# Komputerowe-Projektowanie-Lekow/pmarlo

Measured on AMD Instinct MI355X. Metric: frames/sec featurize->TICA->k-means->T-matrix, 1Mx64 synth; ITS rel-err, higher is better.
Workload: dtype f64; 1 GPU; synthetic 1000000 frames x 64 f32 features per GPU (AR(1) latents), TICA->10, k=500 (10 Lloyd iterations), lag=10, row-normalised T; frames_per_gpu=1000000, features=64, tica_dim=10, k=500, lag=10, kmeans_iters=10, parallelism=shards1

## Files before the change

### pmarlo_amd/csrc/kmeans.hip

```cpp
#include "common.h"
#include "wave.h"

#include <algorithm>
#include <cstdlib>

namespace {

constexpr int kThreads = 256;

template <typename T>
__device__ __forceinline__ double load_as_f64(const T* p) { return (double)(*p); }

struct FitState {
    double scale;
    double inv_scale;
    double absmax;
    double shift2;
    double tol2;
    double done;
    double n_iter;
    double inertia;
};

__device__ __forceinline__ long long to_fixed(double v, double scale) { return __double2ll_rn(v * scale); }
// ... 748 lines not shown
}

__global__ void mfma_f16_probe_kernel(const uint16_t* __restrict__ A, const uint16_t* __restrict__ B,
                                      const float* __restrict__ C, float* __restrict__ D) {
    const int l = threadIdx.x, i = l & 15, q = l >> 4;
    A += (size_t)blockIdx.x * 512;
    B += (size_t)blockIdx.x * 512;
    C += (size_t)blockIdx.x * 256;
    D += (size_t)blockIdx.x * 256;
    v8h a, b;
    for (int j = 0; j < 8; ++j) {
        a[j] = __builtin_bit_cast(_Float16, A[i * 32 + 8 * q + j]);
        b[j] = __builtin_bit_cast(_Float16, B[(8 * q + j) * 16 + i]);
    }
    v4f32 c;
    for (int r = 0; r < 4; ++r) c[r] = C[(4 * q + r) * 16 + i];
    c = __builtin_amdgcn_mfma_f32_16x16x32_f16(a, b, c, 0, 0, 0);
    for (int r = 0; r < 4; ++r) D[(4 * q + r) * 16 + i] = c[r];
}

bool filter_enabled() {
    static const bool on = [] {
        const char* e = getenv("MSM_KMEANS_FILTER");
        return !(e && e[0] == '0');
    }();
    return on;
}

size_t filter_image_bytes(int64_t n, int) { return (size_t)((n + 63) & ~(int64_t)63) * 16 * kFilterRowQ + 16; }

template <typename T>
msm_status launch_pack(msm_ctx* ctx, const T* x, int64_t n, int d, int64_t ld, const double* mean, const double* stdv,
                       const double* absmax, uint4* image) {
    const unsigned grid = (unsigned)((n + 255) / 256);
    if (!absmax) {
        uint4* tail = image + (size_t)((n + 63) & ~(int64_t)63) * kFilterRowQ;
        MSM_HIP(ctx, hipMemsetAsync(tail, 0, 8, ctx->stream));
        const int g = (int)std::min<int64_t>((n * d + 256 * 8 - 1) / (256 * 8), (int64_t)ctx->n_cu * 8);
        hipLaunchKernelGGL(filter_absmax_kernel<T>, dim3(g), dim3(256), 0, ctx->stream, x, n, d, ld, mean, stdv,
                           (unsigned long long*)tail);
        MSM_CHECK_LAUNCH(ctx);
        absmax = (const double*)tail;
    }
    const int dense = ld == d && ((uintptr_t)x & 15) == 0;
#define MSM_PACK_CASE(D)                                                                                              \
    case D:                                                                                                           \
        hipLaunchKernelGGL((kmeans_pack_kernel<T, D>), dim3(grid), dim3(256), 0, ctx->stream, x, n, ld, mean, stdv, absmax, \
                           image, dense);                                                                             \
        break
    switch (d) {
        MSM_PACK_CASE(1); MSM_PACK_CASE(2); MSM_PACK_CASE(3); MSM_PACK_CASE(4); MSM_PACK_CASE(5);
        MSM_PACK_CASE(6); MSM_PACK_CASE(7); MSM_PACK_CASE(8); MSM_PACK_CASE(9); MSM_PACK_CASE(10);
        default: return msm_fail(ctx, MSM_ERR_UNSUPPORTED, "k-means frame images need d <= %d (got %d)", kFilterMaxD, d);
    }
#undef MSM_PACK_CASE
    MSM_CHECK_LAUNCH(ctx);
    return MSM_OK;
}

msm_status filter_stats_buffer(msm_ctx* ctx, unsigned long long** out) {
    static_assert(sizeof(unsigned long long) == 8, "");
    if (!ctx->km_stats) {
        if (ctx->capturing) { *out = nullptr; return MSM_OK; }
        MSM_HIP(ctx, hipMalloc(&ctx->km_stats, 16));
        MSM_HIP(ctx, hipMemsetAsync(ctx->km_stats, 0, 16, ctx->stream));
    }
    *out = (unsigned long long*)ctx->km_stats;
    return MSM_OK;
}

template <typename T, int DP, bool ACCUM>
msm_status launch_filter_dp(msm_ctx* ctx, const T* x, int64_t n, int d, int64_t ld, const double* centers, int k,
                            const double* mean, const double* stdv, const uint4* image, int32_t* labels, double* mindist,
                            const FitState* st, unsigned long long* sums, unsigned long long* counts, double* upd_centers) {
    constexpr int NF = 4;
    const size_t lds = filter_lds_bytes(k, d, ACCUM);
    msm_status rs;
    const int64_t n_units = (n + 16 * NF - 1) / (16 * NF);
    const int kWaves = filter_waves(DP, ACCUM, sizeof(T) == 8 && !mean);
    const int grid = (int)std::min<int64_t>((n_units + kWaves - 1) / kWaves, (int64_t)ctx->n_cu);
    unsigned long long* stats = nullptr;
    rs = filter_stats_buffer(ctx, &stats);
    if (rs != MSM_OK) return rs;
    auto kern = mean ? kmeans_filter_kernel<T, DP, NF, ACCUM, true> : kmeans_filter_kernel<T, DP, NF, ACCUM, false>;
    if (lds > 48 * 1024)
        MSM_HIP(ctx, hipFuncSetAttribute((const void*)kern, hipFuncAttributeMaxDynamicSharedMemorySize, (int)lds));
    hipLaunchKernelGGL(kern, dim3(grid), dim3(64 * kWaves), lds, ctx->stream, x, n, d, ld, k, mean, stdv, image, centers,
                       labels, mindist, st, sums, counts, stats, stats ? upd_centers : nullptr,
                       stats ? (unsigned int*)(stats + 1) : nullptr);
    MSM_CHECK_LAUNCH(ctx);
    return MSM_OK;
}

template <typename T, bool ACCUM>
msm_status launch_filter(msm_ctx* ctx, const T* x, int64_t n, int d, int64_t ld, const double* centers, int k,
                         const double* mean, const double* stdv, const uint4* image, int32_t* labels, double* mindist,
                         const FitState* st, unsigned long long* sums, unsigned long long* counts, double* upd_centers) {
    if (filter_dp(d) == 4)
        return launch_filter_dp<T, 4, ACCUM>(ctx, x, n, d, ld, centers, k, mean, stdv, image, labels, mindist, st, sums,
                                             counts, upd_centers);
    return launch_filter_dp<T, 10, ACCUM>(ctx, x, n, d, ld, centers, k, mean, stdv, image, labels, mindist, st, sums, counts,
                                          upd_centers);
}

bool filter_fits(int k, int d, bool accum) { return filter_enabled() && d <= kFilterMaxD && filter_lds_bytes(k, d, accum) != 0; }

template <typename T, bool ACCUM>
msm_status dispatch_mfma(msm_ctx* ctx, const T* x, int64_t n, int d, int64_t ld, const double* centers, int k,
                         const double* mean, const double* stdv, int32_t* labels, double* mindist, const FitState* st,
                         unsigned long long* sums, unsigned long long* counts, const void* image = nullptr,
                         double* upd_centers = nullptr, bool* folded = nullptr) {
    if (folded) *folded = false;
    if (filter_fits(k, d, ACCUM)) {
        if (getenv("MSM_KMEANS_DEBUG"))
            fprintf(stderr, "msm_kmeans: filter T=%s n=%lld d=%d k=%d ACCUM=%d\n", sizeof(T) == 4 ? "f32" : "f64", (long long)n,
                    d, k, (int)ACCUM);
        if (!image) {
            msm_status rs = msm_reserve_km_image(ctx, filter_image_bytes(n, d));
            if (rs != MSM_OK) return rs;
            rs = launch_pack<T>(ctx, x, n, d, ld, mean, stdv, nullptr, (uint4*)ctx->km_image);
            if (rs != MSM_OK) return rs;
            image = ctx->km_image;
        }
        if (upd_centers && !(ACCUM && (int64_t)k * d <= kUpdateWide && (ctx->km_stats || !ctx->capturing))) upd_centers = nullptr;
        if (folded) *folded = upd_centers != nullptr;
        return launch_filter<T, ACCUM>(ctx, x, n, d, ld, centers, k, mean, stdv, (const uint4*)image, labels, mindist, st,
                                       sums, counts, upd_centers);
    }
#define MSM_MFMA_CASE(KSV) \
    if (d <= 4 * KSV)      \
        return launch_mfma<T, KSV, ACCUM>(ctx, x, n, d, ld, centers, k, mean, stdv, labels, mindist, st, sums, counts)
    MSM_MFMA_CASE(1);
    MSM_MFMA_CASE(2);
    MSM_MFMA_CASE(3);
    MSM_MFMA_CASE(4);
    MSM_MFMA_CASE(6);
    MSM_MFMA_CASE(8);
    MSM_MFMA_CASE(12);
    MSM_MFMA_CASE(16);
    MSM_MFMA_CASE(24);
    MSM_MFMA_CASE(32);
    MSM_MFMA_CASE(48);
    MSM_MFMA_CASE(64);
#undef MSM_MFMA_CASE
    return msm_fail(ctx, MSM_ERR_UNSUPPORTED, "k-means: d=%d > 256 not supported", d);
}

msm_status mfma_probe(msm_ctx* ctx, bool f16, const uint16_t* h_a, const uint16_t* h_b, const float* h_c, float* h_d,
                      int n_tiles) {
    if (!ctx) return MSM_ERR_INVALID;
    MSM_REQUIRE(ctx, n_tiles >= 1 && h_a && h_b && h_c && h_d, "msm_mfma_probe: bad arguments");
    const size_t na = (size_t)n_tiles * 512 * sizeof(uint16_t), nc = (size_t)n_tiles * 256 * sizeof(float);
    msm_status rs = msm_reserve_scratch(ctx, 2 * na + 2 * nc);
    if (rs != MSM_OK) return rs;
    unsigned char* base = (unsigned char*)ctx->scratch;
    uint16_t* d_a = (uint16_t*)base;
    uint16_t* d_b = (uint16_t*)(base + na);
    float* d_c = (float*)(base + 2 * na);
    float* d_d = (float*)(base + 2 * na + nc);
    MSM_HIP(ctx, hipMemcpyAsync(d_a, h_a, na, hipMemcpyHostToDevice, ctx->stream));
    MSM_HIP(ctx, hipMemcpyAsync(d_b, h_b, na, hipMemcpyHostToDevice, ctx->stream));
    MSM_HIP(ctx, hipMemcpyAsync(d_c, h_c, nc, hipMemcpyHostToDevice, ctx->stream));
    if (f16)
        hipLaunchKernelGGL(mfma_f16_probe_kernel, dim3((unsigned)n_tiles), dim3(64), 0, ctx->stream, d_a, d_b, d_c, d_d);
    else
        hipLaunchKernelGGL(mfma_bf16_probe_kernel, dim3((unsigned)n_tiles), dim3(64), 0, ctx->stream, d_a, d_b, d_c, d_d);
    MSM_CHECK_LAUNCH(ctx);
    MSM_HIP(ctx, hipMemcpyAsync(h_d, d_d, nc, hipMemcpyDeviceToHost, ctx->stream));
    MSM_HIP(ctx, hipStreamSynchronize(ctx->stream));
    return MSM_OK;
}

// ... 251 lines not shown
```

### pmarlo_amd/csrc/kmeans_filter.h

```cpp
#pragma once

typedef __bf16 v8bf __attribute__((ext_vector_type(8)));
typedef _Float16 v8h __attribute__((ext_vector_type(8)));
typedef float v4f32 __attribute__((ext_vector_type(4)));

#ifdef MSM_KMF_WAVES
__host__ __device__ constexpr int filter_waves(int, bool, bool) { return MSM_KMF_WAVES; }
#else
__host__ __device__ constexpr int filter_waves(int dp, bool heavy, bool plain) { return dp == 10 && heavy && !plain ? 12 : 16; }
#endif
constexpr int kFilterMaxD = 10;
constexpr int kFilterRowQ = 3;
constexpr double kFilterHi = 1e18;
constexpr double kFilterScaledHi = 16384.0;
constexpr double kF16MinNormal = 6.103515625e-05;
constexpr int kFilterScaleTop = 13;
constexpr double kFilterKappa = 52.0 * 5.9604644775390625e-08;
constexpr float kPickEps = 20.0f * 5.9604644775390625e-08f;
constexpr float kPickFloor = 1e-30f;
constexpr float kUp20 = 1.0f + 9.5367431640625e-07f;
constexpr double kUp20d = 1.0 + 9.5367431640625e-07;

__host__ __device__ inline int filter_scale_exp(double amax) {
    if (!(amax > 0.0) || !(amax <= 1.7976931348623157e308)) return 0;
// ... 157 lines not shown
    auto slot_addr = [&](int i, int sl) { return ((sl >> 3) * 16 + i) * 8 + (sl & 7); };
#pragma unroll
    for (int u = 0; u < kStageRegs; ++u) {
        const int i = lane + 64 * u;
        const int r = stage_row(i, d), f = i - r * d, j = tile * 16 + r;
        if (i < 16 * d && j < k) {
            tab[(size_t)j * S::RF + f] = (float)c[u];
            const double w = ldexp(c[u], ec);
            if (fabs(w) <= kFilterScaledHi) {
                unsigned short ch, cl;
                double tiny = 0.0;
                f16_split2(w, ch, cl, tiny);
                simg[slot_addr(r, filter_slot(0, f))] = ch;
                simg[slot_addr(r, filter_slot(1, f))] = ch;
                simg[slot_addr(r, filter_slot(2, f))] = cl;
            }
        }
    }
    __builtin_amdgcn_fence(__ATOMIC_ACQ_REL, "wavefront");
    int bad_row = 0;
    if (lane < 16) {
        const int j = tile * 16 + lane;
        float* row = tab + (size_t)j * S::RF;
        double h = __builtin_inf();
        if (j < k) {
            double a = 0.0, aw = 0.0, tiny = 0.0;
            bool ok = true;
#pragma unroll
            for (int f = 0; f < DP; ++f) {
                const double cf = rc[f];
                a = fma(cf, cf, a);
                const double w = ldexp(cf, ec);
                ok = ok && fabs(cf) <= kFilterHi && fabs(w) <= kFilterScaledHi;
                if (ok) {
                    aw = fma(w, w, aw);
                    const double r = fabs(w) >= kF16MinNormal ? fabs(w - f16_round(w)) : fabs(w);
                    if (!(r >= kF16MinNormal) || !(fabs(w) >= kF16MinNormal)) tiny += r;
                }
            }
            h = 0.5 * a;
            const double cval = ldexp(-(h - kFilterKappa * h), exc);
            ok = ok && fabs(cval) <= 0x1p100;
            if (!ok) bad_row = 1;
            cz[j] = ok ? f32_up(cval) : 0.0f;
            if (ok)
                simg[slot_addr(lane, kFilterSlotNorm)] =
                    f16_bits(f16_ceil(fmax((kFilterKappa * sqrt(aw) + 2.0 * tiny) * kUp20d, kF16MinNormal)));
            row[DP] = (float)h;
            row[DP + 1] = (float)(sqrt(a) * kUp20d);
        } else {
            cz[j] = -3.0e38f;
            row[DP] = 3.0e38f;
            row[DP + 1] = -3.0e38f;
        }
        hs[j] = h;
    }
    const bool bad = __any(bad_row != 0);
    if (bad && lane == 0) atomicOr(any_bad, 1);
}


template <typename T>
__global__ __launch_bounds__(256) void filter_absmax_kernel(const T* __restrict__ x, int64_t n, int d, int64_t ld,
                                                           const double* __restrict__ mean, const double* __restrict__ stdv,
                                                           unsigned long long* __restrict__ out_bits) {
    double m = 0.0;
    for (int64_t i = (int64_t)blockIdx.x * 256 + threadIdx.x; i < n * d; i += (int64_t)gridDim.x * 256) {
        const int64_t r = i / d;
        const int f = (int)(i - r * d);
        double v = load_as_f64(x + r * ld + f);
        if (mean) v = (v - mean[f]) / stdv[f];
        if (fabs(v) <= kFilterHi) m = fmax(m, fabs(v));
    }
    m = wave_max_f64(m);
    __shared__ double wm[4];
    if ((threadIdx.x & 63) == 0) wm[threadIdx.x >> 6] = m;
    __syncthreads();
    if (threadIdx.x == 0) {
        m = fmax(fmax(wm[0], wm[1]), fmax(wm[2], wm[3]));
        if (m > 0.0) atomicMax(out_bits, (unsigned long long)__double_as_longlong(m));
    }
}

template <typename T, int DP, bool WHITEN>
__device__ __forceinline__ void filter_load_frame(const T* __restrict__ x, int64_t ld, int d, bool vec_rows,
                                                  const double* __restrict__ mean, const double* __restrict__ stdv,
                                                  int64_t t, double (&z)[DP]) {
    const T* row = x + t * ld;
    if (vec_rows) {
        const double2* r2 = reinterpret_cast<const double2*>(row);
#pragma unroll
        for (int f2 = 0; f2 < DP / 2; ++f2) {
            const double2 v = r2[f2];
            z[2 * f2] = v.x;
            z[2 * f2 + 1] = v.y;
        }
    } else {
#pragma unroll
        for (int f = 0; f < DP; ++f) {
            const double v = load_as_f64(row + (f < d ? f : d - 1));
            z[f] = f < d ? v : 0.0;
        }
    }
    if constexpr (WHITEN) {
#pragma unroll
        for (int f = 0; f < DP; ++f) {
            const int fc = f < d ? f : d - 1;
            const double w = (z[f] - mean[fc]) / stdv[fc];
            z[f] = f < d ? w : 0.0;
        }
    }
}

template <int MT>
__device__ __forceinline__ void filter_close_iteration(const unsigned long long* sums, const unsigned long long* counts, int k,
                                                       int d, double* centers, FitState* st) {
    __shared__ double red[16];
    const int tid = threadIdx.x;
    const double inv_scale = st->inv_scale;
    for (int v0 = 0; v0 < 1024; v0 += MT) {
        const int v = v0 + tid;
        if (v < 1024) {
            double acc = 0.0;
            constexpr int CH = 4;
            for (int i0 = v; i0 < k * d; i0 += 1024 * CH) {
                long long cnt[CH], sm[CH];
                double old[CH];
#pragma unroll
                for (int c = 0; c < CH; ++c) {
                    const int i = i0 + c * 1024;
                    cnt[c] = 0;
                    if (i < k * d) {
                        cnt[c] = (long long)__hip_atomic_load(&counts[i / d], __ATOMIC_RELAXED, __HIP_MEMORY_SCOPE_AGENT);
                        sm[c] = (long long)__hip_atomic_load(&sums[i], __ATOMIC_RELAXED, __HIP_MEMORY_SCOPE_AGENT);
                        old[c] = centers[i];
                    }
                }
#pragma unroll
                for (int c = 0; c < CH; ++c)
                    if (cnt[c] > 0) {
                        const double c_new = (double)sm[c] * inv_scale / (double)cnt[c];
                        const double dlt = c_new - old[c];
                        acc = fma(dlt, dlt, acc);
                        centers[i0 + c * 1024] = c_new;
                    }
            }
            for (int off = 32; off > 0; off >>= 1) acc += __shfl_down(acc, off, 64);
            if ((v & 63) == 0) red[v >> 6] = acc;
        }
    }
    __syncthreads();
    if (tid == 0) {
        double t = 0.0;
        for (int i = 0; i < 16; ++i) t += red[i];
        st->shift2 = t;
        st->n_iter += 1.0;
        if (t <= st->tol2) st->done = 1.0;
    }
}

template <typename T, int DP, int NF, bool ACCUM, bool WHITEN>
__global__ __launch_bounds__(64 * filter_waves(DP, ACCUM, sizeof(T) == 8 && !WHITEN)) void kmeans_filter_kernel(
    const T* __restrict__ x, int64_t n, int d, int64_t ld, int k, const double* __restrict__ mean,
    const double* __restrict__ stdv, const uint4* __restrict__ image, const double* __restrict__ centers,
    int32_t* __restrict__ labels,
    double* __restrict__ mindist, const FitState* __restrict__ st, unsigned long long* __restrict__ sums,
    unsigned long long* __restrict__ counts, unsigned long long* __restrict__ n_scanned, double* upd_centers,
    unsigned int* __restrict__ ticket) {
    using S = FilterShape<DP>;
    constexpr int kFilterWaves = filter_waves(DP, ACCUM, sizeof(T) == 8 && !WHITEN);
    constexpr int kMT = 64 * kFilterWaves, RF = S::RF, RQ = kFilterRowQ;
    constexpr bool kReloadZ = ACCUM && DP == 10;
    static_assert(NF == 4, "one frame group per lane quarter: a unit is 64 frames, one per lane in the candidate pick");
    extern __shared__ __attribute__((aligned(16))) unsigned char smem_raw[];
    if constexpr (ACCUM) {
        if (st->done != 0.0) return;
    }
    const int k16 = (k + 15) & ~15;
    const int n_tiles = ((k16 / 16) + 1) & ~1;
    uint4* img = reinterpret_cast<uint4*>(smem_raw);
    float* tab = reinterpret_cast<float*>(img + (size_t)n_tiles * 64);
    float* cz = tab + (size_t)n_tiles * 16 * RF;
    double* hs = reinterpret_cast<double*>(cz + (size_t)n_tiles * 16);
    unsigned long long* lsum = reinterpret_cast<unsigned long long*>(hs + (size_t)n_tiles * 16);
    unsigned long long* lcnt = lsum + (ACCUM ? (size_t)k * d : 0);
    __shared__ int unit_ctr;
    __shared__ int any_bad;
    __shared__ unsigned long long cmax_bits;
    const int tid = threadIdx.x, lane = tid & 63, wave = __builtin_amdgcn_readfirstlane(tid >> 6);
    const int j16 = lane & 15, q = lane >> 4;
    const double scale = ACCUM ? st->scale : 0.0;
    if (tid == 0) {
        unit_ctr = kFilterWaves;
        any_bad = 0;
        cmax_bits = 0ull;
    }
    KSTAMP_INIT
    if constexpr (ACCUM) {
        for (int i = tid; i < k * (d + 1); i += kMT) lsum[i] = 0ull;
    }
    __syncthreads();
    constexpr int kUnit = 16 * NF;
    const int64_t n_units = (n + kUnit - 1) / kUnit;
    const int64_t units_per_block = (n_units + gridDim.x - 1) / gridDim.x;
    const int64_t u_begin = (int64_t)blockIdx.x * units_per_block;
    const int64_t u_end = min(n_units, u_begin + units_per_block);
    const int voff = j16 * RQ + filter_piece(q);
    const int ex = reinterpret_cast<const int*>(image + (size_t)((n + 63) & ~(int64_t)63) * RQ)[2];

    int64_t unit = u_begin + wave;
    v8h b[NF];
    auto load_images = [&](int64_t un) {
        const uint4* ub = image + un * (kUnit * RQ);
#pragma unroll
        for (int u = 0; u < NF; ++u) b[u] = __builtin_bit_cast(v8h, ub[voff + u * 16 * RQ]);
    };
    if constexpr (!kReloadZ) {
        if (unit < u_end) load_images(unit);
    }

    {
        double cm = 0.0;
        for (int i = tid; i < k * d; i += kMT) cm = fmax(cm, fabs(centers[i]));
        cm = wave_max_f64(cm);
        if (lane == 0 && cm > 0.0) atomicMax(&cmax_bits, (unsigned long long)__double_as_longlong(cm));
    }
    __syncthreads();
    const int ec = __builtin_amdgcn_readfirstlane(filter_scale_exp(__longlong_as_double((long long)cmax_bits)));
    const int exc = ex + ec;
    for (int t = wave; t < n_tiles; t += 2 * kFilterWaves) {
        const int t2 = t + kFilterWaves;
        double c0[kStageRegs], c1[kStageRegs], r0[DP], r1[DP];
        filter_stage_fetch<DP>(t, lane, centers, k, d, c0, r0);
        if (t2 < n_tiles) filter_stage_fetch<DP>(t2, lane, centers, k, d, c1, r1);
        filter_stage_build<DP>(t, lane, reinterpret_cast<unsigned short*>(img + (size_t)t * 64), c0, r0, k, d, ec, exc, tab, cz,
                               hs, &any_bad);
        if (t2 < n_tiles)
            filter_stage_build<DP>(t2, lane, reinterpret_cast<unsigned short*>(img + (size_t)t2 * 64), c1, r1, k, d, ec, exc, tab,
                                   cz, hs, &any_bad);
    }
    __syncthreads();
    const float inv_scale_u = __int_as_float((127 - exc) << 23);
    const bool all_scan = __builtin_amdgcn_readfirstlane(any_bad) != 0;
    KSTAMP(0);

    if constexpr (kReloadZ) {
        if (unit < u_end) load_images(unit);
    }
    unsigned long long my_scans = 0;
    const bool vec_rows = sizeof(T) == 8 && d == DP && ((ld * sizeof(T)) & 15) == 0 && (((uintptr_t)x) & 15) == 0;
    const int iters = n_tiles / 2;
    constexpr int kNone = 0x7fffffff;

    auto load_frame = [&](int64_t t, double (&z)[DP]) { filter_load_frame<T, DP, WHITEN>(x, ld, d, vec_rows, mean, stdv, t, z); };
    auto score64 = [&](const double* crow, int c, const double (&z)[DP]) {
        double a = 0.0;
#pragma unroll
        for (int f = 0; f < DP; ++f)
            if (f < d) a = fma(crow[f], z[f], a);
        return a - hs[c];
    };
    auto write_label = [&](int64_t t, int bidx, double bm, const double (&z)[DP]) {
        labels[t] = bidx;
        if (mindist) {
            double zsq = 0.0;
#pragma unroll
            for (int f = 0; f < DP; ++f) zsq = fma(z[f], z[f], zsq);
            const double md = -2.0 * bm + zsq;
            mindist[t] = md > 0.0 ? md : 0.0;
        }
    };
    auto commit_scan = [&](int64_t t, int sbi, double sbest, const double (&zz)[DP], int old_s) {
        if constexpr (ACCUM) {
            if (!labels || old_s != sbi) {
#pragma unroll
                for (int f = 0; f < DP; ++f) {
                    if (f < d && lane == f) {
                        const unsigned long long fx = (unsigned long long)to_fixed(zz[f], scale);
                        atomicAdd(&lsum[(size_t)sbi * d + f], fx);
                        if (old_s >= 0) atomicAdd(&lsum[(size_t)old_s * d + f], 0ull - fx);
                    }
                }
                if (lane == 0) {
                    atomicAdd(&lcnt[sbi], 1ull);
                    if (old_s >= 0) atomicAdd(&lcnt[old_s], ~0ull);
                    if (labels) labels[t] = sbi;
                }
            }
        } else {
            if (lane == 0) write_label(t, sbi, sbest, zz);
        }
    };
    auto scan_frame = [&](int64_t t) {
        double zz[DP];
        load_frame(t, zz);
        double sbest = -__builtin_inf();
        int sbi = kNone;
        for (int c = lane; c < k; c += 64) {
            const double sc = score64(centers + (size_t)c * d, c, zz);
            if (sc > sbest) { sbest = sc; sbi = c; }
        }
#pragma unroll
        for (int off = 1; off < 64; off <<= 1) {
            const double ob = __shfl_xor(sbest, off, 64);
            const int oi = __shfl_xor(sbi, off, 64);
            if (ob > sbest || (ob == sbest && oi < sbi)) { sbest = ob; sbi = oi; }
        }
        if (sbi >= k) { sbi = 0; sbest = -__builtin_inf(); }
        int old_s = -1;
        if constexpr (ACCUM) {
            if (labels) old_s = labels[t];
        }
        commit_scan(t, sbi, sbest, zz, old_s);
#ifdef MSM_KMF_DIAG_COUNT
        if (MSM_KMF_DIAG_COUNT == 1) ++my_scans;
#else
        ++my_scans;
#endif
    };

    while (unit < u_end) {
        int nt = 0;
        if (lane == 0) nt = atomicAdd(&unit_ctr, 1);
        const int64_t nxt = u_begin + __builtin_amdgcn_readfirstlane(nt);
        KSTAMP_VM(1);
        float b1[NF], b2[NF];
        int bp[NF];
#pragma unroll
        for (int u = 0; u < NF; ++u) { b1[u] = -__builtin_inff(); b2[u] = -__builtin_inff(); bp[u] = 0; }
#ifdef MSM_KMF_DIAG_NOTILE
        for (int it = 0; it < (iters < 9 ? iters : 9); ++it) {
#else
        for (int it = 0; it < iters; ++it) {
#endif
            const int jt = 2 * it;
            const v8h aa = __builtin_bit_cast(v8h, img[(jt + 0) * 64 + lane]);
            const v8h ab = __builtin_bit_cast(v8h, img[(jt + 1) * 64 + lane]);
            const v4f32 ca = *reinterpret_cast<const v4f32*>(cz + (jt + 0) * 16 + 4 * q);
            const v4f32 cb = *reinterpret_cast<const v4f32*>(cz + (jt + 1) * 16 + 4 * q);
            v4f32 acca[NF], accb[NF];
#pragma unroll
            for (int u = 0; u < NF; ++u) {
                acca[u] = __builtin_amdgcn_mfma_f32_16x16x32_f16(aa, b[u], ca, 0, 0, 0);
                accb[u] = __builtin_amdgcn_mfma_f32_16x16x32_f16(ab, b[u], cb, 0, 0, 0);
            }
#pragma unroll
            for (int u = 0; u < NF; ++u) {
                float m = max3_f32(b2[u], acca[u][0], acca[u][1]);
                m = max3_f32(m, acca[u][2], acca[u][3]);
                m = max3_f32(m, accb[u][0], accb[u][1]);
                m = max3_f32(m, accb[u][2], accb[u][3]);
                const bool better = m > b1[u];
                b2[u] = med3_f32(b1[u], b2[u], m);
                b1[u] = hw_max_f32(b1[u], m);
                bp[u] = better ? jt : bp[u];
            }
        }
        KSTAMP(2);
        bool guard[NF];
#pragma unroll
        for (int u = 0; u < NF; ++u) guard[u] = q == 3 && __builtin_bit_cast(unsigned short, b[u][7]) == 0x7C00;
        if (nxt < u_end) load_images(nxt);
        const int64_t f0 = unit * kUnit + lane;
        const bool fok = f0 < n;
        const int64_t fr = fok ? f0 : n - 1;
        int old = -1;
        if constexpr (ACCUM) {
            if (labels) old = labels[fr];
        }
        double z[DP];
        load_frame(fr, z);
        int cd = kNone;
        float Ru = __builtin_inff();
#ifdef MSM_KMF_DIAG_NOCROSS
        cd = bp[0] | (q << 16);
        Ru = b2[0] + b1[1] + b1[2] + b1[3] + b2[1] + b2[2] + b2[3] + (guard[0] | guard[1] | guard[2] | guard[3] ? 1.f : 0.f) + (float)(bp[1] + bp[2] + bp[3]);
#else
#pragma unroll
        for (int u = 0; u < NF; ++u) {
            const float M1 = xrow_max_f32(b1[u]);
            const int code_u = xrow_min_i32(b1[u] == M1 ? ((q << 16) | bp[u]) : kNone);
            const int gs = code_u >> 16;
            float r = q == gs ? b2[u] : b1[u];
            if (guard[u]) r = __builtin_inff();
            const float R_u = xrow_max_f32(r);
            cd = q == u ? code_u : cd;
            Ru = q == u ? R_u : Ru;
        }
#endif
        Ru = __builtin_fmaf(Ru, inv_scale_u, 1.40129846e-45f);
        KSTAMP(3);
        const int gs = cd >> 16, pstar = cd & 0xffff;
        const int base = min(pstar * 16 + 4 * gs, n_tiles * 16 - 20);
        float pz[DP];
        float qz = 0.f;
#pragma unroll
        for (int f = 0; f < DP; ++f) {
            pz[f] = (float)z[f];
            qz = __builtin_fmaf(pz[f], pz[f], qz);
        }
        const bool z_bad = !(qz < __builtin_inff());
        const float zn = hw_max_f32(__builtin_amdgcn_sqrtf(qz) * kUp20, 1.0f);
        float s1 = -__builtin_inff(), s2 = -__builtin_inff(), sbmax = 0.f;
        int i1 = 0;
#ifndef MSM_KMF_DIAG_NOPICK
        const float* p_row = tab + (size_t)base * RF;
#pragma unroll
        for (int c = 0; c < 8; ++c) {
            const float4* r4 = reinterpret_cast<const float4*>(p_row + ((c & 3) + 16 * (c >> 2)) * RF);
            float a = 0.f, h, cn;
            if constexpr (DP == 4) {
                const float4 r0 = r4[0], r1 = r4[1];
                a = __builtin_fmaf(r0.x, pz[0], a);
                a = __builtin_fmaf(r0.y, pz[1], a);
                a = __builtin_fmaf(r0.z, pz[2], a);
                a = __builtin_fmaf(r0.w, pz[3], a);
                h = r1.x;
                cn = r1.y;
            } else {
                const float4 r0 = r4[0], r1 = r4[1], r2 = r4[2];
                a = __builtin_fmaf(r0.x, pz[0], a);
                a = __builtin_fmaf(r0.y, pz[1], a);
                a = __builtin_fmaf(r0.z, pz[2], a);
                a = __builtin_fmaf(r0.w, pz[3], a);
                a = __builtin_fmaf(r1.x, pz[4], a);
                a = __builtin_fmaf(r1.y, pz[5], a);
                a = __builtin_fmaf(r1.z, pz[6], a);
                a = __builtin_fmaf(r1.w, pz[7], a);
                a = __builtin_fmaf(r2.x, pz[8], a);
                a = __builtin_fmaf(r2.y, pz[9], a);
                h = r2.z;
                cn = r2.w;
            }
            const float s = a - h;
            sbmax = hw_max_f32(sbmax, __builtin_fmaf(zn, cn, h));
            const bool better = s > s1;
            s2 = med3_f32(s1, s2, s);
            s1 = hw_max_f32(s1, s);
            i1 = better ? c : i1;
        }
#endif
        const float e = __builtin_fmaf(kPickEps, sbmax, kPickFloor);
        const int jw = base + (i1 & 3) + 16 * (i1 >> 2);
        const bool certified = !all_scan && !z_bad && cd != kNone && jw < k && s1 - s2 > 2.0f * e && s1 - e > Ru;
        const int lab = jw;
#if defined(MSM_KMF_DIAG_NOSCAN) || defined(MSM_KMF_DIAG_NOQUEUE)
        unsigned long long todo = 0;
#else
        unsigned long long todo = __ballot(fok && !certified);
#endif
        KSTAMP(4);
#ifdef MSM_KMF_DIAG_NOCOMMIT
        if (fok && certified && cd == 12345) {
#else
        if (fok && certified) {
#endif
            if constexpr (ACCUM) {
                if (!labels || old != lab) {
                    double zm[DP];
                    if constexpr (kReloadZ) {
                        load_frame(f0, zm);
                    } else {
#pragma unroll
                        for (int f = 0; f < DP; ++f) zm[f] = z[f];
                    }
#pragma unroll
                    for (int f = 0; f < DP; ++f) {
                        if (f < d) {
                            const unsigned long long fx = (unsigned long long)to_fixed(zm[f], scale);
                            atomicAdd(&lsum[(size_t)lab * d + f], fx);
                            if (old >= 0) atomicAdd(&lsum[(size_t)old * d + f], 0ull - fx);
                        }
                    }
                    atomicAdd(&lcnt[lab], 1ull);
                    if (old >= 0) atomicAdd(&lcnt[old], ~0ull);
                    if (labels) labels[f0] = lab;
                }
            } else {
                if (mindist) write_label(f0, lab, score64(centers + (size_t)lab * d, lab, z), z);
                else labels[f0] = lab;
            }
        }
        KSTAMP(5);
        while (todo) {
            const int jf = __builtin_ctzll(todo);
            todo &= todo - 1;
            const int64_t t = ((int64_t)__builtin_amdgcn_readlane((int)(f0 >> 32), jf) << 32) |
                              (unsigned)__builtin_amdgcn_readlane((int)f0, jf);
            const bool plain = all_scan || __builtin_amdgcn_readlane((int)(z_bad || !(Ru < __builtin_inff())), jf) != 0;
            if (plain) {
                scan_frame(t);
                continue;
            }
            float zf[DP];
#pragma unroll
            for (int f = 0; f < DP; ++f) zf[f] = __int_as_float(__builtin_amdgcn_readlane(__float_as_int(pz[f]), jf));
            const float znj = __int_as_float(__builtin_amdgcn_readlane(__float_as_int(zn), jf));
            float t1 = -__builtin_inff(), t2 = -__builtin_inff(), t3 = -__builtin_inff(), sbl = 0.f;
            int c1 = 0, c2 = 0;
            for (int c = lane; c < n_tiles * 16; c += 64) {
                const float4* r4 = reinterpret_cast<const float4*>(tab + (size_t)c * RF);
                float a = 0.f, h, cn;
                if constexpr (DP == 4) {
                    const float4 r0 = r4[0], r1 = r4[1];
                    a = __builtin_fmaf(r0.x, zf[0], a);
                    a = __builtin_fmaf(r0.y, zf[1], a);
                    a = __builtin_fmaf(r0.z, zf[2], a);
                    a = __builtin_fmaf(r0.w, zf[3], a);
                    h = r1.x;
                    cn = r1.y;
                } else {
                    const float4 r0 = r4[0], r1 = r4[1], r2 = r4[2];
                    a = __builtin_fmaf(r0.x, zf[0], a);
                    a = __builtin_fmaf(r0.y, zf[1], a);
                    a = __builtin_fmaf(r0.z, zf[2], a);
                    a = __builtin_fmaf(r0.w, zf[3], a);
                    a = __builtin_fmaf(r1.x, zf[4], a);
                    a = __builtin_fmaf(r1.y, zf[5], a);
                    a = __builtin_fmaf(r1.z, zf[6], a);
                    a = __builtin_fmaf(r1.w, zf[7], a);
                    a = __builtin_fmaf(r2.x, zf[8], a);
                    a = __builtin_fmaf(r2.y, zf[9], a);
                    h = r2.z;
                    cn = r2.w;
                }
                const float sc = a - h;
                sbl = hw_max_f32(sbl, __builtin_fmaf(znj, cn, h));
                if (sc > t1) { t3 = t2; t2 = t1; c2 = c1; t1 = sc; c1 = c; }
                else if (sc > t2) { t3 = t2; t2 = sc; c2 = c; }
                else t3 = hw_max_f32(t3, sc);
            }
            double rowa[DP], rowb[DP];
            {
                const double* ca = centers + (size_t)(c1 < k ? c1 : 0) * d;
                const double* cb = centers + (size_t)(c2 < k ? c2 : 0) * d;
#pragma unroll
                for (int f = 0; f < DP; ++f) {
                    rowa[f] = f < d ? ca[f] : 0.0;
                    rowb[f] = f < d ? cb[f] : 0.0;
                }
            }
            double zz[DP];
            if constexpr (kReloadZ) load_frame(t, zz);
            const float top = wave_max_f32(t1), sbw = wave_max_f32(sbl);
            const float band = top - 2.0f * __builtin_fmaf(kPickEps, sbw, kPickFloor);
            const unsigned long long in1 = __ballot(t1 >= band);
            if (__any(t3 >= band) || in1 == 0ull) {
                scan_frame(t);
                continue;
            }
            if constexpr (!kReloadZ) {
#pragma unroll
                for (int f = 0; f < DP; ++f) {
                    const long long bits = __double_as_longlong(z[f]);
                    zz[f] = __longlong_as_double((long long)(((unsigned long long)(unsigned)__builtin_amdgcn_readlane((int)(bits >> 32), jf) << 32) |
                                                             (unsigned)__builtin_amdgcn_readlane((int)bits, jf)));
                }
            }
            const int old_t = __builtin_amdgcn_readlane(old, jf);
            int sbi;
            double sbest = 0.0;
            const bool two = __any(t2 >= band) || __builtin_popcountll(in1) > 1;
            if (!two && !(mindist && !ACCUM)) {
                sbi = __builtin_amdgcn_readlane(c1, __builtin_ctzll(in1));
            } else {
                double m1 = -__builtin_inf();
                int i1b = kNone;
                auto chain = [&](const double (&row)[DP], int c) {
                    double a = 0.0;
#pragma unroll
                    for (int f = 0; f < DP; ++f) a = fma(row[f], zz[f], a);
                    return a - hs[c];
                };
                if (t1 >= band && c1 < k) { m1 = chain(rowa, c1); i1b = c1; }
                if (t2 >= band && c2 < k) {
                    const double m2 = chain(rowb, c2);
                    if (m2 > m1 || (m2 == m1 && c2 < i1b)) { m1 = m2; i1b = c2; }
                }
                sbest = wave_max_f64(m1);
                sbi = wave_min_i32(m1 == sbest ? i1b : kNone);
                if (sbi >= k) {
                    scan_frame(t);
                    continue;
                }
            }
            commit_scan(t, sbi, sbest, zz, old_t);
#ifdef MSM_KMF_DIAG_COUNT
            if (MSM_KMF_DIAG_COUNT == 2 && two) ++my_scans;
#else
            ++my_scans;
#endif
        }
        KSTAMP(6);
        unit = nxt;
    }
    KSTAMP(7);
    if (n_scanned && lane == 0 && my_scans) atomicAdd(n_scanned, my_scans);
    if constexpr (ACCUM) {
        __syncthreads();
        for (int i = tid; i < k * d; i += kMT)
            if (lsum[i]) atomicAdd(&sums[i], lsum[i]);
        for (int i = tid; i < k; i += kMT)
            if (lcnt[i]) atomicAdd(&counts[i], lcnt[i]);
        if (upd_centers) {
            __shared__ int is_last;
            asm volatile("s_waitcnt vmcnt(0)" ::: "memory");
            __syncthreads();
            if (tid == 0) {
                const unsigned t = __hip_atomic_fetch_add(ticket, 1u, __ATOMIC_RELAXED, __HIP_MEMORY_SCOPE_AGENT);
                is_last = t == gridDim.x - 1;
                if (is_last) __hip_atomic_store(ticket, 0u, __ATOMIC_RELAXED, __HIP_MEMORY_SCOPE_AGENT);
            }
            __syncthreads();
            if (is_last) filter_close_iteration<kMT>(sums, counts, k, d, upd_centers, const_cast<FitState*>(st));
        }
    }
    KSTAMP_FLUSH
}

static inline size_t filter_lds_bytes(int k, int d, bool accum) {
    if (d > kFilterMaxD) return 0;
    const int k16 = (k + 15) & ~15;
    const int n_tiles = ((k16 / 16) + 1) & ~1;
    const size_t tile_bytes = filter_dp(d) == 4 ? FilterShape<4>::kTileBytes : FilterShape<10>::kTileBytes;
    const size_t total = (size_t)n_tiles * tile_bytes + (accum ? (size_t)k * (d + 1) * sizeof(unsigned long long) : 0);
    const size_t cap = 160 * 1024 - 64;
    return total <= cap ? total : 0;
}
```

Measured before the change: 732.8 million frames/s.

## Cut register pressure in k-means filter kernel via 32-bit indexing and kernarg packing

Rarely used pointers (mindist, sums, counts, n_scanned, upd_centers, ticket) are packed into a struct read lazily through the kernarg segment pointer. Per-block base pointers allow 32-bit frame and unit indices, with a host-side guard that rejects shards too large for that. Loop invariants are pinned to scalar registers with asm barriers, and the pick-stage table rows are prefetched a couple of iterations ahead in some configurations. The aim is fewer VGPRs/SGPRs and less 64-bit address arithmetic in the hot loop, in exchange for a frame-count limit and more fragile compiler-coaxing code.

```diff
diff --git a/pmarlo_amd/csrc/kmeans.hip b/pmarlo_amd/csrc/kmeans.hip
--- a/pmarlo_amd/csrc/kmeans.hip
+++ b/pmarlo_amd/csrc/kmeans.hip
@@ -854,12 +854,15 @@
     unsigned long long* stats = nullptr;
     rs = filter_stats_buffer(ctx, &stats);
     if (rs != MSM_OK) return rs;
+    if ((n_units + grid - 1) / grid > (int64_t)(INT32_MAX / (16 * NF)))
+        return msm_fail(ctx, MSM_ERR_UNSUPPORTED, "k-means filter: %lld frames per shard are too many", (long long)n);
     auto kern = mean ? kmeans_filter_kernel<T, DP, NF, ACCUM, true> : kmeans_filter_kernel<T, DP, NF, ACCUM, false>;
     if (lds > 48 * 1024)
         MSM_HIP(ctx, hipFuncSetAttribute((const void*)kern, hipFuncAttributeMaxDynamicSharedMemorySize, (int)lds));
-    hipLaunchKernelGGL(kern, dim3(grid), dim3(64 * kWaves), lds, ctx->stream, x, n, d, ld, k, mean, stdv, image, centers,
-                       labels, mindist, st, sums, counts, stats, stats ? upd_centers : nullptr,
-                       stats ? (unsigned int*)(stats + 1) : nullptr);
+    const FilterRare rare{mindist, sums, counts, stats, stats ? upd_centers : nullptr,
+                          stats ? (unsigned int*)(stats + 1) : nullptr};
+    hipLaunchKernelGGL(kern, dim3(grid), dim3(64 * kWaves), lds, ctx->stream, rare, x, n, d, ld, k, mean, stdv, image, centers,
+                       labels, st);
     MSM_CHECK_LAUNCH(ctx);
     return MSM_OK;
 }
diff --git a/pmarlo_amd/csrc/kmeans_filter.h b/pmarlo_amd/csrc/kmeans_filter.h
--- a/pmarlo_amd/csrc/kmeans_filter.h
+++ b/pmarlo_amd/csrc/kmeans_filter.h
@@ -263,11 +263,20 @@
     }
 }
 
+struct FilterRare {
+    double* mindist;
+    unsigned long long* sums;
+    unsigned long long* counts;
+    unsigned long long* n_scanned;
+    double* upd_centers;
+    unsigned int* ticket;
+};
+
 template <typename T, int DP, bool WHITEN>
 __device__ __forceinline__ void filter_load_frame(const T* __restrict__ x, int64_t ld, int d, bool vec_rows,
                                                   const double* __restrict__ mean, const double* __restrict__ stdv,
-                                                  int64_t t, double (&z)[DP]) {
-    const T* row = x + t * ld;
+                                                  int t, double (&z)[DP]) {
+    const T* row = x + (int64_t)t * ld;
     if (vec_rows) {
         const double2* r2 = reinterpret_cast<const double2*>(row);
 #pragma unroll
@@ -279,8 +288,8 @@
     } else {
 #pragma unroll
         for (int f = 0; f < DP; ++f) {
-            const double v = load_as_f64(row + (f < d ? f : d - 1));
-            z[f] = f < d ? v : 0.0;
+            z[f] = 0.0;
+            if (f < d) z[f] = load_as_f64(row + f);
         }
     }
     if constexpr (WHITEN) {
@@ -342,12 +351,11 @@
 
 template <typename T, int DP, int NF, bool ACCUM, bool WHITEN>
 __global__ __launch_bounds__(64 * filter_waves(DP, ACCUM, sizeof(T) == 8 && !WHITEN)) void kmeans_filter_kernel(
-    const T* __restrict__ x, int64_t n, int d, int64_t ld, int k, const double* __restrict__ mean,
-    const double* __restrict__ stdv, const uint4* __restrict__ image, const double* __restrict__ centers,
-    int32_t* __restrict__ labels,
-    double* __restrict__ mindist, const FitState* __restrict__ st, unsigned long long* __restrict__ sums,
-    unsigned long long* __restrict__ counts, unsigned long long* __restrict__ n_scanned, double* upd_centers,
-    unsigned int* __restrict__ ticket) {
+    const FilterRare rare_in_kernarg, const T* __restrict__ x, int64_t n, int d, int64_t ld, int k,
+    const double* __restrict__ mean, const double* __restrict__ stdv, const uint4* __restrict__ image,
+    const double* __restrict__ centers, int32_t* __restrict__ labels, const FitState* __restrict__ st) {
+    const FilterRare* rare = (const FilterRare*)__builtin_amdgcn_kernarg_segment_ptr();
+    double* const mindist = ACCUM ? nullptr : rare->mindist;
     using S = FilterShape<DP>;
     constexpr int kFilterWaves = filter_waves(DP, ACCUM, sizeof(T) == 8 && !WHITEN);
     constexpr int kMT = 64 * kFilterWaves, RF = S::RF, RQ = kFilterRowQ;
@@ -386,18 +394,25 @@
     const int64_t units_per_block = (n_units + gridDim.x - 1) / gridDim.x;
     const int64_t u_begin = (int64_t)blockIdx.x * units_per_block;
     const int64_t u_end = min(n_units, u_begin + units_per_block);
+    const int n_mine = u_end > u_begin ? (int)(u_end - u_begin) : 0;
+    const int64_t fb0 = u_begin * kUnit;
+    const int nb = n_mine ? (int)min(n - fb0, (int64_t)n_mine * kUnit) : 0;
+    const T* const xb = x + fb0 * ld;
+    const uint4* const imgb = image + u_begin * (kUnit * RQ);
+    int32_t* const labb = labels ? labels + fb0 : nullptr;
+    double* const mdb = mindist ? mindist + fb0 : nullptr;
     const int voff = j16 * RQ + filter_piece(q);
     const int ex = reinterpret_cast<const int*>(image + (size_t)((n + 63) & ~(int64_t)63) * RQ)[2];
 
-    int64_t unit = u_begin + wave;
+    int unit = wave;
     v8h b[NF];
-    auto load_images = [&](int64_t un) {
-        const uint4* ub = image + un * (kUnit * RQ);
+    auto load_images = [&](int un) {
+        const uint4* ub = imgb + (int64_t)un * (kUnit * RQ);
 #pragma unroll
         for (int u = 0; u < NF; ++u) b[u] = __builtin_bit_cast(v8h, ub[voff + u * 16 * RQ]);
     };
     if constexpr (!kReloadZ) {
-        if (unit < u_end) load_images(unit);
+        if (unit < n_mine) load_images(unit);
     }
 
     {
@@ -421,64 +436,65 @@
                                    cz, hs, &any_bad);
     }
     __syncthreads();
-    const float inv_scale_u = __int_as_float((127 - exc) << 23);
-    const bool all_scan = __builtin_amdgcn_readfirstlane(any_bad) != 0;
     KSTAMP(0);
 
     if constexpr (kReloadZ) {
-        if (unit < u_end) load_images(unit);
+        if (unit < n_mine) load_images(unit);
     }
     unsigned long long my_scans = 0;
     const bool vec_rows = sizeof(T) == 8 && d == DP && ((ld * sizeof(T)) & 15) == 0 && (((uintptr_t)x) & 15) == 0;
-    const int iters = n_tiles / 2;
     constexpr int kNone = 0x7fffffff;
-
-    auto load_frame = [&](int64_t t, double (&z)[DP]) { filter_load_frame<T, DP, WHITEN>(x, ld, d, vec_rows, mean, stdv, t, z); };
+    int dv = d, ntv = n_tiles, excv = exc, badv = __builtin_amdgcn_readfirstlane(any_bad), nbv = nb, qv = q;
+    int has_lab = __builtin_amdgcn_readfirstlane(labels != nullptr);
+
+    auto load_frame = [&](int t, double (&z)[DP]) { filter_load_frame<T, DP, WHITEN>(xb, ld, dv, vec_rows, mean, stdv, t, z); };
     auto score64 = [&](const double* crow, int c, const double (&z)[DP]) {
         double a = 0.0;
 #pragma unroll
         for (int f = 0; f < DP; ++f)
-            if (f < d) a = fma(crow[f], z[f], a);
+            if (f < dv) a = fma(crow[f], z[f], a);
         return a - hs[c];
     };
-    auto write_label = [&](int64_t t, int bidx, double bm, const double (&z)[DP]) {
-        labels[t] = bidx;
-        if (mindist) {
+    auto write_label = [&](int t, int bidx, double bm, const double (&z)[DP]) {
+        labb[t] = bidx;
+        if (mdb) {
             double zsq = 0.0;
 #pragma unroll
             for (int f = 0; f < DP; ++f) zsq = fma(z[f], z[f], zsq);
             const double md = -2.0 * bm + zsq;
-            mindist[t] = md > 0.0 ? md : 0.0;
+            mdb[t] = md > 0.0 ? md : 0.0;
         }
     };
-    auto commit_scan = [&](int64_t t, int sbi, double sbest, const double (&zz)[DP], int old_s) {
+    auto commit_scan = [&](int t, int sbi, double sbest, const double (&zz)[DP], int old_s) {
         if constexpr (ACCUM) {
-            if (!labels || old_s != sbi) {
+            if (!has_lab || old_s != sbi) {
+                int ln = lane;
+                asm volatile("" : "+v"(ln));
 #pragma unroll
                 for (int f = 0; f < DP; ++f) {
-                    if (f < d && lane == f) {
+                    if (f < dv && ln == f) {
                         const unsigned long long fx = (unsigned long long)to_fixed(zz[f], scale);
-                        atomicAdd(&lsum[(size_t)sbi * d + f], fx);
-                        if (old_s >= 0) atomicAdd(&lsum[(size_t)old_s * d + f], 0ull - fx);
+                        atomicAdd(&lsum[(size_t)sbi * dv + f], fx);
+                        if (old_s >= 0) atomicAdd(&lsum[(size_t)old_s * dv + f], 0ull - fx);
                     }
                 }
                 if (lane == 0) {
                     atomicAdd(&lcnt[sbi], 1ull);
                     if (old_s >= 0) atomicAdd(&lcnt[old_s], ~0ull);
-                    if (labels) labels[t] = sbi;
+                    if (has_lab) labb[t] = sbi;
                 }
             }
         } else {
             if (lane == 0) write_label(t, sbi, sbest, zz);
         }
     };
-    auto scan_frame = [&](int64_t t) {
+    auto scan_frame = [&](int t) {
         double zz[DP];
         load_frame(t, zz);
         double sbest = -__builtin_inf();
         int sbi = kNone;
         for (int c = lane; c < k; c += 64) {
-            const double sc = score64(centers + (size_t)c * d, c, zz);
+            const double sc = score64(centers + (size_t)c * dv, c, zz);
             if (sc > sbest) { sbest = sc; sbi = c; }
         }
 #pragma unroll
@@ -490,7 +506,7 @@
         if (sbi >= k) { sbi = 0; sbest = -__builtin_inf(); }
         int old_s = -1;
         if constexpr (ACCUM) {
-            if (labels) old_s = labels[t];
+            if (has_lab) old_s = labb[t];
         }
         commit_scan(t, sbi, sbest, zz, old_s);
 #ifdef MSM_KMF_DIAG_COUNT
@@ -500,10 +516,15 @@
 #endif
     };
 
-    while (unit < u_end) {
+    while (unit < n_mine) {
+        asm volatile("" : "+s"(dv), "+s"(ntv), "+s"(excv), "+s"(badv), "+s"(nbv), "+v"(qv));
+        const bool all_scan = badv != 0;
+        const float inv_scale_u = __int_as_float((127 - excv) << 23);
+        const int iters = ntv / 2;
+        const float* const tabv = reinterpret_cast<const float*>(img + ntv * 64);
         int nt = 0;
         if (lane == 0) nt = atomicAdd(&unit_ctr, 1);
-        const int64_t nxt = u_begin + __builtin_amdgcn_readfirstlane(nt);
+        const int nxt = __builtin_amdgcn_readfirstlane(nt);
         KSTAMP_VM(1);
         float b1[NF], b2[NF];
         int bp[NF];
@@ -540,39 +561,43 @@
         KSTAMP(2);
         bool guard[NF];
 #pragma unroll
-        for (int u = 0; u < NF; ++u) guard[u] = q == 3 && __builtin_bit_cast(unsigned short, b[u][7]) == 0x7C00;
-        if (nxt < u_end) load_images(nxt);
-        const int64_t f0 = unit * kUnit + lane;
-        const bool fok = f0 < n;
-        const int64_t fr = fok ? f0 : n - 1;
+        for (int u = 0; u < NF; ++u) {
+            unsigned gw = __builtin_bit_cast(uint4, b[u]).w;
+            asm volatile("" : "+v"(gw));
+            guard[u] = qv == 3 && (gw >> 16) == 0x7C00u;
+        }
+        load_images(nxt < n_mine ? nxt : unit);
+        const int f0 = unit * kUnit + lane;
+        const bool fok = f0 < nbv;
+        const int fr = fok ? f0 : nbv - 1;
         int old = -1;
         if constexpr (ACCUM) {
-            if (labels) old = labels[fr];
+            if (has_lab) old = labb[fr];
         }
         double z[DP];
         load_frame(fr, z);
         int cd = kNone;
         float Ru = __builtin_inff();
 #ifdef MSM_KMF_DIAG_NOCROSS
-        cd = bp[0] | (q << 16);
+        cd = bp[0] | (qv << 16);
         Ru = b2[0] + b1[1] + b1[2] + b1[3] + b2[1] + b2[2] + b2[3] + (guard[0] | guard[1] | guard[2] | guard[3] ? 1.f : 0.f) + (float)(bp[1] + bp[2] + bp[3]);
 #else
 #pragma unroll
         for (int u = 0; u < NF; ++u) {
             const float M1 = xrow_max_f32(b1[u]);
-            const int code_u = xrow_min_i32(b1[u] == M1 ? ((q << 16) | bp[u]) : kNone);
+            const int code_u = xrow_min_i32(b1[u] == M1 ? ((qv << 16) | bp[u]) : kNone);
             const int gs = code_u >> 16;
-            float r = q == gs ? b2[u] : b1[u];
+            float r = qv == gs ? b2[u] : b1[u];
             if (guard[u]) r = __builtin_inff();
             const float R_u = xrow_max_f32(r);
-            cd = q == u ? code_u : cd;
-            Ru = q == u ? R_u : Ru;
+            cd = qv == u ? code_u : cd;
+            Ru = qv == u ? R_u : Ru;
         }
 #endif
         Ru = __builtin_fmaf(Ru, inv_scale_u, 1.40129846e-45f);
         KSTAMP(3);
         const int gs = cd >> 16, pstar = cd & 0xffff;
-        const int base = min(pstar * 16 + 4 * gs, n_tiles * 16 - 20);
+        const int base = min(pstar * 16 + 4 * gs, ntv * 16 - 20);
         float pz[DP];
         float qz = 0.f;
 #pragma unroll
@@ -585,13 +610,22 @@
         float s1 = -__builtin_inff(), s2 = -__builtin_inff(), sbmax = 0.f;
         int i1 = 0;
 #ifndef MSM_KMF_DIAG_NOPICK
-        const float* p_row = tab + (size_t)base * RF;
+        const float* p_row = tabv + base * RF;
+        constexpr int kRowQ = RF / 4, kPickAhead = (kReloadZ || DP == 4) ? 2 : 0;
+        float4 rows[8][kRowQ];
+        auto fetch_row = [&](int c) {
+            const float4* r4 = reinterpret_cast<const float4*>(p_row + ((c & 3) + 16 * (c >> 2)) * RF);
+#pragma unroll
+            for (int i = 0; i < kRowQ; ++i) rows[c][i] = r4[i];
+        };
+#pragma unroll
+        for (int c = 0; c < kPickAhead; ++c) fetch_row(c);
 #pragma unroll
         for (int c = 0; c < 8; ++c) {
-            const float4* r4 = reinterpret_cast<const float4*>(p_row + ((c & 3) + 16 * (c >> 2)) * RF);
+            if (c + kPickAhead < 8) fetch_row(c + kPickAhead);
             float a = 0.f, h, cn;
             if constexpr (DP == 4) {
-                const float4 r0 = r4[0], r1 = r4[1];
+                const float4 r0 = rows[c][0], r1 = rows[c][1];
                 a = __builtin_fmaf(r0.x, pz[0], a);
                 a = __builtin_fmaf(r0.y, pz[1], a);
                 a = __builtin_fmaf(r0.z, pz[2], a);
@@ -599,7 +633,7 @@
                 h = r1.x;
                 cn = r1.y;
             } else {
-                const float4 r0 = r4[0], r1 = r4[1], r2 = r4[2];
+                const float4 r0 = rows[c][0], r1 = rows[c][1], r2 = rows[c][2];
                 a = __builtin_fmaf(r0.x, pz[0], a);
                 a = __builtin_fmaf(r0.y, pz[1], a);
                 a = __builtin_fmaf(r0.z, pz[2], a);
@@ -637,7 +671,7 @@
         if (fok && certified) {
 #endif
             if constexpr (ACCUM) {
-                if (!labels || old != lab) {
+                if (!has_lab || old != lab) {
                     double zm[DP];
                     if constexpr (kReloadZ) {
                         load_frame(f0, zm);
@@ -647,27 +681,26 @@
                     }
 #pragma unroll
                     for (int f = 0; f < DP; ++f) {
-                        if (f < d) {
+                        if (f < dv) {
                             const unsigned long long fx = (unsigned long long)to_fixed(zm[f], scale);
-                            atomicAdd(&lsum[(size_t)lab * d + f], fx);
-                            if (old >= 0) atomicAdd(&lsum[(size_t)old * d + f], 0ull - fx);
+                            atomicAdd(&lsum[(size_t)lab * dv + f], fx);
+                            if (old >= 0) atomicAdd(&lsum[(size_t)old * dv + f], 0ull - fx);
                         }
                     }
                     atomicAdd(&lcnt[lab], 1ull);
                     if (old >= 0) atomicAdd(&lcnt[old], ~0ull);
-                    if (labels) labels[f0] = lab;
+                    if (has_lab) labb[f0] = lab;
                 }
             } else {
-                if (mindist) write_label(f0, lab, score64(centers + (size_t)lab * d, lab, z), z);
-                else labels[f0] = lab;
+                if (mdb) write_label(f0, lab, score64(centers + (size_t)lab * dv, lab, z), z);
+                else labb[f0] = lab;
             }
         }
         KSTAMP(5);
         while (todo) {
             const int jf = __builtin_ctzll(todo);
             todo &= todo - 1;
-            const int64_t t = ((int64_t)__builtin_amdgcn_readlane((int)(f0 >> 32), jf) << 32) |
-                              (unsigned)__builtin_amdgcn_readlane((int)f0, jf);
+            const int t = __builtin_amdgcn_readlane(f0, jf);
             const bool plain = all_scan || __builtin_amdgcn_readlane((int)(z_bad || !(Ru < __builtin_inff())), jf) != 0;
             if (plain) {
                 scan_frame(t);
@@ -679,8 +712,8 @@
             const float znj = __int_as_float(__builtin_amdgcn_readlane(__float_as_int(zn), jf));
             float t1 = -__builtin_inff(), t2 = -__builtin_inff(), t3 = -__builtin_inff(), sbl = 0.f;
             int c1 = 0, c2 = 0;
-            for (int c = lane; c < n_tiles * 16; c += 64) {
-                const float4* r4 = reinterpret_cast<const float4*>(tab + (size_t)c * RF);
+            for (int c = lane; c < ntv * 16; c += 64) {
+                const float4* r4 = reinterpret_cast<const float4*>(tabv + c * RF);
                 float a = 0.f, h, cn;
                 if constexpr (DP == 4) {
                     const float4 r0 = r4[0], r1 = r4[1];
@@ -713,12 +746,12 @@
             }
             double rowa[DP], rowb[DP];
             {
-                const double* ca = centers + (size_t)(c1 < k ? c1 : 0) * d;
-                const double* cb = centers + (size_t)(c2 < k ? c2 : 0) * d;
+                const double* ca = centers + (size_t)(c1 < k ? c1 : 0) * dv;
+                const double* cb = centers + (size_t)(c2 < k ? c2 : 0) * dv;
 #pragma unroll
                 for (int f = 0; f < DP; ++f) {
-                    rowa[f] = f < d ? ca[f] : 0.0;
-                    rowb[f] = f < d ? cb[f] : 0.0;
+                    rowa[f] = f < dv ? ca[f] : 0.0;
+                    rowb[f] = f < dv ? cb[f] : 0.0;
                 }
             }
             double zz[DP];
@@ -742,7 +775,7 @@
             int sbi;
             double sbest = 0.0;
             const bool two = __any(t2 >= band) || __builtin_popcountll(in1) > 1;
-            if (!two && !(mindist && !ACCUM)) {
+            if (!two && !(mdb && !ACCUM)) {
                 sbi = __builtin_amdgcn_readlane(c1, __builtin_ctzll(in1));
             } else {
                 double m1 = -__builtin_inf();
@@ -776,8 +809,12 @@
         unit = nxt;
     }
     KSTAMP(7);
+    unsigned long long* n_scanned = rare->n_scanned;
     if (n_scanned && lane == 0 && my_scans) atomicAdd(n_scanned, my_scans);
     if constexpr (ACCUM) {
+        unsigned long long* sums = rare->sums;
+        unsigned long long* counts = rare->counts;
+        double* upd_centers = rare->upd_centers;
         __syncthreads();
         for (int i = tid; i < k * d; i += kMT)
             if (lsum[i]) atomicAdd(&sums[i], lsum[i]);
@@ -788,9 +825,9 @@
             asm volatile("s_waitcnt vmcnt(0)" ::: "memory");
             __syncthreads();
             if (tid == 0) {
-                const unsigned t = __hip_atomic_fetch_add(ticket, 1u, __ATOMIC_RELAXED, __HIP_MEMORY_SCOPE_AGENT);
+                const unsigned t = __hip_atomic_fetch_add(rare->ticket, 1u, __ATOMIC_RELAXED, __HIP_MEMORY_SCOPE_AGENT);
                 is_last = t == gridDim.x - 1;
-                if (is_last) __hip_atomic_store(ticket, 0u, __ATOMIC_RELAXED, __HIP_MEMORY_SCOPE_AGENT);
+                if (is_last) __hip_atomic_store(rare->ticket, 0u, __ATOMIC_RELAXED, __HIP_MEMORY_SCOPE_AGENT);
             }
             __syncthreads();
             if (is_last) filter_close_iteration<kMT>(sums, counts, k, d, upd_centers, const_cast<FitState*>(st));
```

Measured after the change: 734.3 million frames/s (median of 5 runs). Within noise of the previous version (+0.2%).
